# songlab-cal/CherryML

Hardware: AMD Instinct MI355X
Metric: cherry-pairs/sec (whole node) per EM iter (higher is better)
Workload: dtype f64

## Files before the change

### cherryml_amd/csrc/cb_internal.hip.h

```cpp
#pragma once
#include "../../include/cherrybank.h"

#include <hip/hip_runtime.h>

#include <algorithm>
#include <atomic>
#include <chrono>
#include <cmath>
#include <cstdarg>
#include <cstdio>
#include <cstdlib>
#include <cstring>
#include <string>
#include <vector>

int cb_fail(int code, const char *fmt, ...);
#define fail cb_fail

#define HIP_TRY(expr)                                                                   \
  do {                                                                                  \
    hipError_t e_ = (expr);                                                             \
    if (e_ != hipSuccess)                                                               \
      return fail(e_ == hipErrorOutOfMemory ? CB_ENOMEM : CB_EHIP, "%s failed: %s (%s:%d)", \
                  #expr, hipGetErrorString(e_), __FILE__, __LINE__);                    \
  } while (0)

#define CB_REUSE_EIGH 256
int cb_internal_expm_bank(cb_handle h, const double *Q, const double *pi, int flags, double *P);
int cb_internal_set_times(cb_handle h, const double *t_host, int B, const double *t_dev);
struct CbSpectral {
  int S = 0, LD = 0;
  const double *A = nullptr, *U = nullptr, *lam = nullptr, *dsq = nullptr, *sigma = nullptr;
};
int cb_internal_spectral(cb_handle h, CbSpectral *out);

int cb_launch_bank_fused(int variant, int kg, const void *args, int grid, hipStream_t stream, hipEvent_t stop);

#define CB_TB_RS_MAX 24
#define CB_TB_RG_MAX 40
struct CbTimeBasisHost {
  int B = 0, ns = 0, nd = 0, ng = 0;
  double rho_max = 0.0;
  double res_s = 0.0, res_g = 0.0;
  std::vector<int> kind;
  std::vector<int> skel_s, direct, skel_g;
  std::vector<double> tf, tg;
  std::vector<double> Ls, Lg;
};
bool cb_tb_build(int B, const double *t, double rho_max, CbTimeBasisHost &out);
struct CbTbEwArgs {
  int S, LD, B, ns, nd, ng;
  int nsmall;
  const double *Ct;
  const double *Psi;
  const double *A;
  const double *t;
  const double *Ls, *Lg;
  double *Gh;
  float *Gh32;
  double *loss_part;
  double inv_n;
  const unsigned long long *skip;
};
int cb_tb_launch_tables(int LD, int ns, int nd, int ng, const double *tf, const double *tg, const double *lam, double *F, double *E,
                        double *H, const unsigned long long *skip, hipStream_t stream);
#define CB_TB_LDS_MAX (144u << 10)
size_t cb_tb_ew_lds_bytes(int B, int ns, int ng);
bool cb_tb_supported(int B, int LD, int ns, int ng);
int cb_tb_prepare_ew(int B, int ns, int ng, size_t *cache);
int cb_tb_launch_ew(const CbTbEwArgs &a, hipStream_t stream, hipEvent_t stop, int *nparts);

static inline const char *cb_test_hook(const char *name) {
  const char *on = getenv("CB_TEST_HOOKS");
  return (on && on[0] == '1') ? getenv(name) : nullptr;
}
static inline size_t cb_hook_bytes(const char *name, size_t bytes) {
  const char *s = cb_test_hook(name);
  const long long x = s ? atoll(s) : 0;
  return x > 0 ? (size_t)x : bytes;
}

struct CbDevBufs {
  std::vector<void *> ptrs;
  ~CbDevBufs() {
    for (void *p : ptrs)
      if (p) (void)hipFree(p);
  }
  template <typename T>
  T *up(const T *host, size_t count, int &rc) {
    void *q = nullptr;
    if (rc != CB_OK) return nullptr;
    if (hipMalloc(&q, (count ? count : 1) * sizeof(T)) != hipSuccess) {
      rc = fail(CB_ENOMEM, "device allocation failed");
      return nullptr;
    }
    ptrs.push_back(q);
// ... 56 lines not shown
```

### cherryml_amd/csrc/cherrybank.hip

```cpp
#include "cb_internal.hip.h"

#include "common.hip.h"
#include "jacobi_block.hip.h"
#include "jacobi_wave.hip.h"
#include "large_bank.hip.h"
#include "small_bank.hip.h"
#include "train_small.hip.h"
#include "train_large.hip.h"
#include "general_small.hip.h"
#include "general_large.hip.h"
#include "eigh_planned.hip.h"

#define CB_ABI_VERSION 2

static thread_local std::string g_err;

int cb_fail(int code, const char *fmt, ...) {
  char buf[512];
  va_list ap;
  va_start(ap, fmt);
  vsnprintf(buf, sizeof buf, fmt, ap);
  va_end(ap);
  g_err = buf;
  return code;
// ... 204 lines not shown
      return nb;
    });
    h->tb_next_pending = true;
    h->tb_next_epoch = epoch + lead;
  }
  return CB_OK;
}

struct LargeBankForm {
  bool tb = false;
  bool fused = false;
  bool accum = false;
  int kg = 1;
  int n_parts = 1;
  int tiles_k3 = 0;
  int test_no_claim = 0;
  double phi_delta = 0;
};

static LargeBankForm choose_large_form(const cb_bank *h, int B, bool Pd, bool want_grad, bool planned_now) {
  static const int streams = getenv("CB_BANK_STREAMS") ? std::min(4, std::max(1, atoi(getenv("CB_BANK_STREAMS")))) : 1;
  const char *tb_hook = cb_test_hook("CB_BANK_TB"), *fused_hook = cb_test_hook("CB_BANK_FUSED"),
             *unfused_hook = cb_test_hook("CB_BANK_UNFUSED"), *k3_hook = cb_test_hook("CB_BANK_K3"),
             *kg_hook = cb_test_hook("CB_BANK_KG"), *no_claim_hook = cb_test_hook("CB_BANK_TEST_NO_CLAIM"),
             *phi_z_hook = cb_test_hook("CB_PHI_Z");
  const int LD = h->LD, tm = (LD + LG_TM - 1) / LG_TM, tn = (LD + LG_TN - 1) / LG_TN;
  const bool f32 = h->dtype == CB_F32 && !Pd;
  LargeBankForm f;
  const bool form_hooks = fused_hook || unfused_hook || k3_hook || kg_hook || no_claim_hook;
  f.tb = h->sym_counts && !h->per_bucket_products && !h->tb_block && !h->tb_failed && !Pd && want_grad && h->tb_Ls[0] &&
         streams == 1 && (h->dtype == CB_F64 || h->dtype == CB_MIXED) &&
         (tb_hook ? atoi(tb_hook) != 0 : (!form_hooks && B >= CB_TB_MIN_B));
  if (f.tb && planned_now && h->tb.B != B) f.tb = false;
  {
    const size_t nb16 = (size_t)LD / 16, cap = (size_t)B * tm * tn;
    if (nb16 * (nb16 + 1) > cap) f.tb = false;
  }
  f.fused = !Pd && want_grad && !unfused_hook && streams == 1 && h->bank_queue && (fused_hook || B >= CB_BANK_FUSED_MIN_B);
  f.accum = h->sym_counts && !h->per_bucket_products && !Pd && want_grad && h->Yk && streams == 1 && h->dtype == CB_F64 &&
            (k3_hook ? atoi(k3_hook) == 0 : (B >= CB_BANK_SUM_FIRST_MIN_B && h->phi_delta >= 4e-3));
  f.tiles_k3 = f.accum ? 0 : h->sym_counts ? tn * (tn + 1) / 2 : tm * tn;
  f.phi_delta = h->phi_delta;
  if (phi_z_hook) f.phi_delta *= atof(phi_z_hook) / 0.1;
  f.kg = (B < CB_BANK_KG2_MAX_B && !f32) ? 2 : 1;
  if (kg_hook) f.kg = atoi(kg_hook) == 1 ? 1 : 2;
  if (Pd) f.kg = 1;
  if (streams > 1 && h->dtype == CB_F64 && !Pd && want_grad && B >= 4 * streams && !h->comm && !h->profile) f.n_parts = streams;
  f.test_no_claim = no_claim_hook ? 1 : 0;
  return f;
}

struct LargeCall {
  int B;
  const double *t;
  double inv_n;
  double *loss, *dQ, *Pd;
  bool dA_padded, planned_now;
  const unsigned long long *skipw;
  size_t LL;
  int tiles, tiles_k1;
};

template <typename T1, typename TG>
struct BankBufs {
  const T1 *Ut, *A, *F, *Ct;
  TG *Gt, *T;
  const TG *U;
  int variant;
};
template <typename T1, typename TG>
// ... 38 lines not shown
                        hipEvent_t k3_stop) {
  const int LD = h->LD;
  const LossArgs la{h->loss_part, nparts, h->S, h->dsq, h->dirsum, c.inv_n, c.loss, c.skipw};
  const dim3 red_grid((unsigned)((c.LL + 255) / 256) + 1);
  if (f.accum) {
    hipLaunchKernelGGL(ky_reduce_loss<TG>, red_grid, dim3(256), 0, h->stream, src, YArgs{LD, c.B, c.t, h->E, h->Yk}, la);
    K4Args gl{h->S, LD, h->Yk, h->U, h->Lk, nullptr, nullptr, nullptr};
    gl.skip = c.skipw;
    gl.ystride = c.LL;
    launch_sg(h, gl, 0, 0.0, 0.0, nullptr, nullptr, 1 + CB_PHI_TERMS);
    LAUNCH_STOP(k3_stop, kphi_combine<CB_PHI_TERMS>, dim3((unsigned)((c.LL + 255) / 256)), dim3(256), 0, h->stream, LD, h->Lk,
                h->lam, f.phi_delta, h->Mt, c.skipw);
  } else {
    hipLaunchKernelGGL(k3_reduce_loss<TG>, red_grid, dim3(256), 0, h->stream, src, nb, c.LL, h->Mt, sym_ld, la);
  }
  enqueue_k4(h, c, c.skipw, stop_event(h, EV_K4));
  HIP_TRY(hipGetLastError());
  return CB_OK;
}

template <typename TG>
static int enqueue_tb_bank(cb_bank *h, const LargeBankForm &f, const LargeCall &c) {
  constexpr bool mixed = std::is_same_v<TG, float>;
  const CbTimeBasisHost &bas = h->tb;
  const int S = h->S, LD = h->LD, set = h->tb_set, nf = bas.ns + bas.nd, ng = bas.ng;
  const auto bb = bank_bufs<double, TG>(h);
  if (!c.planned_now && cb_tb_launch_tables(LD, bas.ns, bas.nd, ng, h->tb_tf[set], h->tb_tg[set], h->lam, h->F, h->E, h->H,
                                            c.skipw, h->stream) != 0)
    return fail(CB_EHIP, "tb_tables: launch failed");
  double *psi_buf = mixed ? reinterpret_cast<double *>(h->T32) : h->T;
  K1Args<double> k1{S, LD, nf, h->Vc, h->A, h->tb_tf[set], h->F, h->sigma, h->Ct, psi_buf, h->loss_part, c.inv_n, h->dsq, nullptr, c.skipw};
  LAUNCH_STOP(stop_event(h, EV_K1), (k1_pt_loss_gt<double, double, false, 1, true>), dim3(c.tiles_k1 * nf), dim3(LG4_THREADS), 0,
              h->stream, k1);
  const CbTbEwArgs ew{S, LD, c.B, bas.ns, bas.nd, ng, c.B - bas.nd, h->Ct, psi_buf, h->A, c.t, h->tb_Ls[set], h->tb_Lg[set], h->Gt,
                      mixed ? h->Gt32 : nullptr, h->loss_part, c.inv_n, c.skipw};
  int ew_parts = 0;
  if (cb_tb_launch_ew(ew, h->stream, stop_event(h, EV_K2), &ew_parts) != 0) return fail(CB_EHIP, "tb_ew: launch failed");
  if (mixed) launch_cast_f32(h, c, 0);
  const K2Args<TG> k2{LD, bb.Gt, bb.U, bb.T, c.skipw};
  const K3Args<TG> k3{LD, ng, bb.T, bb.U, h->tb_tg[set], h->lam, h->E, h->H, bb.Gt, 1, c.skipw};
  hipLaunchKernelGGL((k2_t_eq_g_u<TG, 1>), dim3(c.tiles * ng), dim3(LG4_THREADS), 0, h->stream, k2);
  LAUNCH_STOP(stop_event(h, EV_K3), (k3_w_phi<TG, 1>), dim3(c.tiles_k1 * ng), dim3(LG4_THREADS), 0, h->stream, k3);
  return enqueue_tail<TG>(h, f, c, bb.Gt, ng, ew_parts, LD, nullptr);
}

template <typename T1, typename TG>
static int enqueue_fused_bank(cb_bank *h, const LargeBankForm &f, const LargeCall &c) {
  const int S = h->S, LD = h->LD, B = c.B;
  const auto bb = bank_bufs<T1, TG>(h);
  const int total = B * (c.tiles_k1 + c.tiles + f.tiles_k3), grid = std::min(h->bank_slots / f.kg, total);
  const int sym = h->sym_counts ? 1 : 0;
  if (h->profile && h->profile_now) h->ev_rec[EV_K1] = h->ev_rec[EV_K2] = false;
  const hipEvent_t bank_stop = stop_event(h, EV_K3);
  static_assert(sizeof(K123Args<float, float>) == sizeof(K123Args<double, double>) &&
                sizeof(K123Args<double, float>) == sizeof(K123Args<double, double>), "one argument block for all");
  const K123Args<T1, TG> a{{S, LD, B, bb.Ut, bb.A, c.t, bb.F, h->sigma, bb.Ct, bb.Gt, h->loss_part, c.inv_n, h->dsq, nullptr, c.skipw},
                           {LD, bb.Gt, bb.U, bb.T, c.skipw},
                           {LD, B, bb.T, bb.U, c.t, h->lam, h->E, h->H, bb.Gt, sym, c.skipw},
                           {h->bank_queue, B, c.tiles_k1, c.tiles, f.tiles_k3, h->bank_claims, f.test_no_claim}};
  auto *dst = reinterpret_cast<K123Args<T1, TG> *>(h->bank_args);
  hipLaunchKernelGGL((lg_tables<K123Args<T1, TG>>), dim3((unsigned)(((size_t)B * LD + 255) / 256)), dim3(256), 0, h->stream, LD, B,
                     c.t, h->lam, h->sigma, h->F, h->E, h->H, a, dst, grid);
  if (std::is_same_v<TG, float>) launch_cast_f32(h, c, (size_t)B * LD);
  if (cb_launch_bank_fused(bb.variant, f.kg, dst, grid, h->stream, bank_stop) != 0) return fail(CB_EHIP, "k123_bank: launch failed");
  return enqueue_tail<TG>(h, f, c, f.accum ? bb.T : bb.Gt, B, B * c.tiles_k1, h->sym_counts ? LD : 0, nullptr);
}

// ... 447 lines not shown
```

### cherryml_amd/csrc/create_host.hip.h

```cpp
#pragma once
__global__ void prep_counts(int S, int B, const double *C, double *n, double *inv_n, double *ones,
                            double *dirsum) {
  extern __shared__ double sm[];
  const int l = blockIdx.x;
  const double *Cl = C + (size_t)l * B * S * S;
  for (int e = threadIdx.x; e < S * S; e += blockDim.x) {
    double acc = 0.0;
    for (int b = 0; b < B; ++b) acc += Cl[(size_t)b * S * S + e];
    sm[e] = acc;
  }
  __syncthreads();
  for (int k = threadIdx.x; k < S; k += blockDim.x) {
    double cs = 0.0, rs = 0.0;
    for (int i = 0; i < S; ++i) {
      cs += sm[i * S + k];
      rs += sm[k * S + i];
    }
    dirsum[(size_t)l * S + k] = cs - rs;
  }
  if (threadIdx.x == 0) {
    double tot = 0.0;
    for (int e = 0; e < S * S; ++e) tot += sm[e];
    n[l] = tot;
    inv_n[l] = 1.0 / tot;
// ... 253 lines not shown
      (void)hipMemsetAsync(flag, 0, sizeof(int), h->stream);
      hipLaunchKernelGGL(small_sym_check, dim3((unsigned)nmat), dim3(256), 0, h->stream, S, Cdev, flag);
      int hf = 1;
      if (hipMemcpyAsync(&hf, flag, sizeof hf, hipMemcpyDeviceToHost, h->stream) == hipSuccess &&
          hipStreamSynchronize(h->stream) == hipSuccess)
        h->sym_counts = hf == 0 && !cb_test_hook("CB_NO_SYM");
      (void)hipMemsetAsync(flag, 0, sizeof(int), h->stream);
    }
  } else {
    const size_t LL = (size_t)h->LD * h->LD;
    const int tiles = ((h->LD + LG_TM - 1) / LG_TM) * ((h->LD + LG_TN - 1) / LG_TN);
    h->k3_chunk = 4;
    h->k3_nchunks = (B + h->k3_chunk - 1) / h->k3_chunk;
    double *tot = nullptr;
    const bool f32 = h->dtype == CB_F32, mixed = h->dtype == CB_MIXED, narrow = f32 || mixed;
    const size_t per_bucket = (expm_only || narrow) ? 0 : (size_t)Bl * LL;
    const size_t per_bucket32 = narrow ? (size_t)Bl * LL : 0;
    bool ok = dev_alloc(h, &h->Ct, mixed ? (size_t)Bl * LL : per_bucket) == CB_OK && dev_alloc(h, &tot, SS) == CB_OK &&
              dev_alloc(h, &h->Ct32, f32 ? per_bucket32 : 0) == CB_OK && dev_alloc(h, &h->Gt32, per_bucket32) == CB_OK &&
              dev_alloc(h, &h->T32, per_bucket32) == CB_OK && dev_alloc(h, &h->Uf, narrow ? LL : 0) == CB_OK &&
              dev_alloc(h, &h->Utf, narrow ? LL : 0) == CB_OK && dev_alloc(h, &h->Af, narrow ? LL : 0) == CB_OK &&
              dev_alloc(h, &h->Ff, narrow ? (size_t)B * h->LD : 0) == CB_OK &&
              dev_alloc(h, &h->A, LL) == CB_OK && dev_alloc(h, &h->dsq, h->LD) == CB_OK &&
              dev_alloc(h, &h->Gc, LL) == CB_OK && dev_alloc(h, &h->Vc, LL) == CB_OK &&
              dev_alloc(h, &h->Gc2, LL) == CB_OK && dev_alloc(h, &h->gx, 12 * LL + (size_t)h->LD + 16 + 3 * 256 + 8) == CB_OK &&
              dev_alloc(h, &h->U, LL) == CB_OK && dev_alloc(h, &h->lam, h->LD) == CB_OK &&
              dev_alloc(h, &h->sigma, 8) == CB_OK && dev_alloc(h, &h->off_bits, 64) == CB_OK &&
              dev_alloc(h, &h->F, (size_t)B * h->LD) == CB_OK &&
              dev_alloc(h, &h->E, (size_t)B * h->LD) == CB_OK &&
              dev_alloc(h, &h->H, (size_t)B * h->LD) == CB_OK &&
              dev_alloc(h, &h->Gt, per_bucket) == CB_OK &&
              dev_alloc(h, &h->T, per_bucket) == CB_OK &&
              dev_alloc(h, &h->Mt, LL) == CB_OK && dev_alloc(h, &h->X, LL) == CB_OK &&
              dev_alloc(h, &h->loss_part, (size_t)B * tiles) == CB_OK &&
              dev_alloc(h, &h->Yk, expm_only ? 0 : (1 + CB_PHI_TERMS) * LL) == CB_OK &&
              dev_alloc(h, &h->Lk, expm_only ? 0 : (1 + CB_PHI_TERMS) * LL) == CB_OK;
    if (ok && !expm_only && !f32)
      for (int k = 0; k < 2 && ok; ++k)
        ok = dev_alloc(h, &h->tb_Ls[k], (size_t)Bl * CB_TB_RS_MAX) == CB_OK && dev_alloc(h, &h->tb_Lg[k], (size_t)Bl * CB_TB_RG_MAX) == CB_OK &&
             dev_alloc(h, &h->tb_tf[k], Bl) == CB_OK && dev_alloc(h, &h->tb_tg[k], Bl) == CB_OK;
    if (!ok) {
      free_tmp();
      return cleanup(CB_ENOMEM);
    }
    {
      void *q = nullptr;
      if (hipHostMalloc(&q, 8 * sizeof(unsigned long long), hipHostMallocCoherent | hipHostMallocMapped) == hipSuccess) {
        h->poll = (unsigned long long *)q;
        memset(q, 0, 8 * sizeof(unsigned long long));
      } else {
        (void)hipGetLastError();
      }
    }
    if (!expm_only) {
      int dev = 0, cus = 0;
      if (hipGetDevice(&dev) != hipSuccess || hipDeviceGetAttribute(&cus, hipDeviceAttributeMultiprocessorCount, dev) != hipSuccess)
        cus = 256;
      h->bank_slots = 4 * std::max(cus, 1);
      h->bank_claims = (h->bank_slots + LG_NQ - 1) / LG_NQ;
      if (dev_alloc(h, &h->bank_queue, (size_t)LG_NQ + 2 * (size_t)B + (size_t)LG_NQ * h->bank_claims) != CB_OK ||
          dev_alloc(h, &h->bank_args, sizeof(K123Args<double, double>)) != CB_OK) {
        free_tmp();
        return cleanup(CB_ENOMEM);
      }
    }
    if (!expm_only) {
    hipLaunchKernelGGL(prep_counts_large_tot, dim3((unsigned)((SS + 255) / 256)), dim3(256), 0,
                       h->stream, S, B, Cdev, tot);
    hipLaunchKernelGGL(prep_counts_large_fin, dim3(1), dim3(256), 0, h->stream, S, tot, h->n_dev,
                       h->inv_n, h->ones, h->dirsum);
    const int nt32 = (h->LD + 31) / 32;
    if (f32) hipLaunchKernelGGL(lg_transpose_pad<float>, dim3(nt32, nt32, Bl), dim3(32, 8), 0, h->stream, S, h->LD,
                                Cdev, h->Ct32, src_idx);
    else hipLaunchKernelGGL(lg_transpose_pad<double>, dim3(nt32, nt32, Bl), dim3(32, 8), 0, h->stream, S, h->LD,
                            Cdev, h->Ct, src_idx);
    {
      int *flag = reinterpret_cast<int *>(h->status);
      (void)hipMemsetAsync(flag, 0, sizeof(int), h->stream);
      if (f32) hipLaunchKernelGGL(lg_sym_check<float>, dim3(nt32, nt32, Bl), dim3(32, 32), 0, h->stream, h->LD, h->Ct32, flag);
      else hipLaunchKernelGGL(lg_sym_check<double>, dim3(nt32, nt32, Bl), dim3(32, 32), 0, h->stream, h->LD, h->Ct, flag);
      int hf = 1;
      if (hipMemcpyAsync(&hf, flag, sizeof hf, hipMemcpyDeviceToHost, h->stream) == hipSuccess &&
          hipStreamSynchronize(h->stream) == hipSuccess)
        h->sym_counts = hf == 0 && !cb_test_hook("CB_NO_SYM");
    }
    }
  }
  h->n_host.resize(L);
  hipError_t e = hipMemcpyAsync(h->n_host.data(), h->n_dev, L * sizeof(double), hipMemcpyDeviceToHost,
                                h->stream);
  if (e == hipSuccess) e = hipStreamSynchronize(h->stream);
  if (Ctmp) (void)hipFree(Ctmp);
  if (e != hipSuccess) return cleanup(fail(CB_EHIP, "cb_create: upload failed: %s", hipGetErrorString(e)));
  e = hipGetLastError();
  if (e != hipSuccess) return cleanup(fail(CB_EHIP, "cb_create: kernel failed: %s", hipGetErrorString(e)));
  for (int l = 0; l < L; ++l)
    if (!(h->n_host[l] > 0.0) || !std::isfinite(h->n_host[l]))
      return cleanup(fail(CB_ENUMERIC, "cb_create: site %d has total count %g", l, h->n_host[l]));
  *out = h;
  return CB_OK;
#undef TRY_ALLOC
#undef TRY_HIP
}

extern "C" void cb_destroy(cb_handle h) {
  if (!h) return;
  if (h->tb_next_pending) (void)h->tb_next.get();
  (void)hipSetDevice(h->dev);
  if (h->own_stream) (void)hipStreamSynchronize(h->own_stream);
  for (hipEvent_t e : h->ev)
    if (e) (void)hipEventDestroy(e);
  for (hipEvent_t e : h->ev2)
    if (e) (void)hipEventDestroy(e);
  for (void *p : h->allocs) (void)hipFree(p);
  for (double *p : h->ws_ptr)
    if (p) (void)hipFree(p);
  if (h->pin) (void)hipHostFree(h->pin);
  if (h->poll) (void)hipHostFree(h->poll);
// ... 13 lines not shown
```

### cherryml_amd/csrc/handle_host.hip.h

```cpp
#pragma once
#include <hip/hip_ext.h>
#include <future>
struct EighSlot {
  int cap = 12;
  int nsq = 0;
  int band_after = 0;
  int so = 0;
  int expect_run = 1, expect_order = 12, expect_sq = 2;
};
struct EighPlan {
  int lead_band = 1;
  int nslots = 0;
  EighSlot slot[EC_MAXREC];
};
struct cb_bank {
  int dev = 0, S = 0, L = 0, B = 0;
  int B_cap = 0;
  hipStream_t xstream[3] = {};
  hipEvent_t ev_fork = nullptr, ev_join[3] = {};
  int tr_epochs = 0;
  uint64_t tr_sig = 0;
  int last_form = 0;
  double tr_pow_b1 = 1.0, tr_pow_b2 = 1.0;
  int dtype = CB_F64;
// ... 31 lines not shown
         *sigma = nullptr, *F = nullptr, *E = nullptr, *H = nullptr, *Gt = nullptr, *T = nullptr,
         *Mt_part = nullptr, *Mt = nullptr, *X = nullptr, *loss_part = nullptr;
  float *Ct32 = nullptr, *Gt32 = nullptr, *T32 = nullptr, *Uf = nullptr, *Utf = nullptr, *Af = nullptr, *Ff = nullptr;
  unsigned long long *off_bits = nullptr;
  unsigned long long *poll = nullptr;
  unsigned long long poll_seq = 0;
  unsigned long long *ectl = nullptr, *epin = nullptr;
  double *epart = nullptr;
  bool begin_folded = false;
  double *sigma_home = nullptr;
  double *sigma2 = nullptr;
  unsigned long long eseq = 0;
  bool planned_unavailable = false;
  int planned_solves = 0, planned_stalls = 0;
  long long record_spins = 0;
  std::vector<double> epoch_seconds;
  EighPlan eplan;
  int k3_chunk = 0, k3_nchunks = 0;
  double *Yk = nullptr, *Lk = nullptr;
  double phi_delta = 0.0;
  unsigned int *bank_queue = nullptr;
  unsigned char *bank_args = nullptr;
  int bank_slots = 0;
  int bank_claims = 0;
  bool bank_fused = false;
  int bank_kg = 1;
  bool bank_accum = false;
  CbTimeBasisHost tb;
  int tb_set = 0;
  double *tb_Ls[2] = {}, *tb_Lg[2] = {}, *tb_tf[2] = {}, *tb_tg[2] = {};
  std::future<CbTimeBasisHost> tb_next;
  bool tb_next_pending = false;
  int tb_next_epoch = 0;
  size_t tb_ew_lds[4] = {0, 0, 0, 0};
  int tb_builds = 0, tb_stale_epochs = 0;
  bool tb_failed = false;
  bool tb_block = false;
  bool bank_tb = false;
  int last_sweeps = 0;
  double *gn_scratch = nullptr, *gn_partial = nullptr;
  int gn_nw = 0;
  struct {
    double *Qn = nullptr, *QT = nullptr, *colsum = nullptr, *alpha = nullptr, *R = nullptr, *RT = nullptr, *E = nullptr,
           *ET = nullptr, *G = nullptr, *GT = nullptr, *Xbar = nullptr, *lpart = nullptr;
    int *nsq = nullptr;
    int cap_slots = 0;
  } gl;
  std::vector<double> t_host, t_live_host;
  bool have_prev = false;
  double *ws_ptr[16] = {};
  size_t ws_cap[16] = {};
  char *pin = nullptr;
  size_t pin_cap = 0, pin_off = 0;
  bool profile = false;
  int profile_every = 1;
  bool profile_now = false;
  hipEvent_t ev[CB_T_COUNT + 1] = {};
  bool ev_rec[CB_T_COUNT + 1] = {};
  double t_sum[CB_T_COUNT] = {};
  int t_calls = 0;
  bool t_pending = false;
  hipEvent_t ev2[CB_T_COUNT + 1] = {};
  bool ev_rec2[CB_T_COUNT + 1] = {};
  bool t_pending2 = false;
};

// ... 102 lines not shown
```

### cherryml_amd/csrc/tbasis.hip.h

```cpp
#pragma once
#include "cb_internal.hip.h"
#include "common.hip.h"
#include <hip/hip_ext.h>

namespace tbasis {

typedef long double ld;

static inline ld g_phi2(ld x) {
  if (fabsl(x) < 0.5L) {
    ld p = 1.0L;
    for (int k = 24; k >= 3; --k) p = 1.0L + p * x / (ld)k;
    return 0.5L * p;
  }
  return (expm1l(x) - x) / (x * x);
}

static inline ld dot4(const ld *a, const ld *b, int n) {
  ld s0 = 0.0L, s1 = 0.0L, s2 = 0.0L, s3 = 0.0L;
  int i = 0;
  for (; i + 3 < n; i += 4) {
    s0 += a[i] * b[i];
    s1 += a[i + 1] * b[i + 1];
    s2 += a[i + 2] * b[i + 2];
    s3 += a[i + 3] * b[i + 3];
  }
  for (; i < n; ++i) s0 += a[i] * b[i];
  return (s0 + s1) + (s2 + s3);
}

static int id_rows(int B, int N, const std::vector<ld> &F, int Rmax, ld tol, std::vector<int> &skel, std::vector<ld> &L, ld &resid) {
  std::vector<ld> W(F), Q((size_t)Rmax * N, 0.0L), Cq((size_t)B * Rmax, 0.0L), q(N);
  skel.clear();
  ld scale = 0.0L;
  int R = 0;
// ... 123 lines not shown
    out.res_g = (double)res;
    out.skel_g = sk;
    for (int b = 0; b < B; ++b)
      for (int r = 0; r < R; ++r)
        out.Lg[(size_t)b * CB_TB_RG_MAX + r] = (double)(L[(size_t)b * R + r] * (ld)t[b] / (ld)t[sk[r]]);
  }
  for (int r = 0; r < out.ns; ++r) out.tf.push_back(t[out.skel_s[r]]);
  for (int r = 0; r < out.nd; ++r) out.tf.push_back(t[out.direct[r]]);
  for (int r = 0; r < out.ng; ++r) out.tg.push_back(t[out.skel_g[r]]);
  return true;
}

__global__ void tb_tables(int LD, int ns, int nd, int ng, const double *__restrict__ tf, const double *__restrict__ tg,
                          const double *__restrict__ lam, double *__restrict__ F, double *__restrict__ E, double *__restrict__ H,
                          const unsigned long long *skip) {
  if (skip && *skip != 0ull) return;
  const int idx = blockIdx.x * blockDim.x + threadIdx.x;
  const int nf = ns + nd;
  if (idx >= (nf + ng) * LD) return;
  const int r = idx / LD, k = idx - r * LD;
  if (r < nf) {
    const double t = tf[r], x = t * lam[k];
    F[idx] = r < ns ? phi2(x) / (t * t) : exp(x);
  } else {
    const double x = tg[r - nf] * lam[k];
    E[idx - nf * LD] = exp(x);
    H[idx - nf * LD] = exp(0.5 * x);
  }
}

template <int RS, int RG>
struct TbEwLds {
  static constexpr int SS = RS + 1, SG = RG + 2;
  int BP, LS, LG, TT, LT, RED, TOTAL;
  __host__ __device__ explicit TbEwLds(int B) {
    BP = (B + 15) & ~15;
    LS = 0;
    LG = LS + BP * SS;
    TT = LG + BP * SG;
    LT = TT + BP;
    RED = LT + 256;
    TOTAL = RED + 16;
  }
};

template <int RS, int RG>
__device__ __forceinline__ void tb_ew_step(int b0, int j, int k, int nsm, const double *sLs, const double *sLg, const double *sT,
                                           const double *ltab, const double (&psi)[RS / 4], double a_e, double dl, double inv_n,
                                           const double (&c)[4], const double (&pd)[4], d4 (&D)[RG / 16], double &loss, int &bad) {
  typedef TbEwLds<RS, RG> Lds;
  const bool any_small = b0 < nsm, any_direct = b0 + 16 > nsm;
  double P[4];
  if (any_small) {
    d4 acc = {0.0, 0.0, 0.0, 0.0};
#ifndef TB_NO_FWD
#pragma unroll
    for (int q = 0; q < RS / 4; ++q) acc = mfma_f64(sLs[(b0 + j) * Lds::SS + 4 * q + k], psi[q], acc);
#endif
#pragma unroll
    for (int m = 0; m < 4; ++m) {
      const double t = sT[b0 + k + 4 * m];
      P[m] = fma(t, fma(t, acc[m], a_e), dl);
    }
    if (any_direct) {
#pragma unroll
      for (int m = 0; m < 4; ++m) P[m] = (b0 + k + 4 * m < nsm) ? P[m] : pd[m];
    }
  } else {
#pragma unroll
    for (int m = 0; m < 4; ++m) P[m] = pd[m];
  }
  double g[4];
#pragma unroll
  for (int m = 0; m < 4; ++m) {
    const double cv = c[m];
    bad |= (!(P[m] >= 1e-300) && cv != 0.0) ? 1 : 0;
    const double Pu = fmax(P[m], 1e-300);
#ifdef TB_NO_LOG
    loss = fma(-cv, Pu, loss);
    g[m] = (-cv * inv_n) * Pu;
#else
    loss = fma(-cv, fast_log_table_unchecked(Pu, ltab), loss);
    g[m] = (-cv * inv_n) * fast_rcp(Pu);
#endif
  }
#ifdef TB_NO_BWD
#pragma unroll
  for (int m = 0; m < 4; ++m) D[0][m] += g[m];
#else
#pragma unroll
  for (int m = 0; m < 4; ++m) {
    const double *w = sLg + (b0 + 4 * m + k) * Lds::SG + j;
#pragma unroll
    for (int q = 0; q < RG / 16; ++q) D[q] = mfma_f64(w[16 * q], g[m], D[q]);
  }
#endif
}

template <int RS, int RG, int NWAVE, bool SYM>
__global__ __launch_bounds__(NWAVE * 64, 4) void tb_ew(CbTbEwArgs a) {
  constexpr int NT = NWAVE * 64;
  typedef TbEwLds<RS, RG> Lds;
  extern __shared__ double smem[];
  if (a.skip && *a.skip != 0ull) return;
  const Lds o(a.B);
  double *sLs = smem + o.LS, *sLg = smem + o.LG, *sT = smem + o.TT, *ltab = smem + o.LT, *sred = smem + o.RED;
  const int tid = threadIdx.x;
  for (int i = tid; i < o.BP * RS; i += NT) {
    const int b = i / RS, r = i - b * RS;
    sLs[b * Lds::SS + r] = b < a.B ? a.Ls[(size_t)b * CB_TB_RS_MAX + r] : 0.0;
  }
  for (int i = tid; i < o.BP * RG; i += NT) {
    const int b = i / RG, r = i - b * RG;
    sLg[b * Lds::SG + r] = (b < a.B && r < CB_TB_RG_MAX) ? a.Lg[(size_t)b * CB_TB_RG_MAX + r] : 0.0;
  }
  for (int i = tid; i < o.BP; i += NT) sT[i] = i < a.B ? a.t[i] : 0.0;
  fast_log_table_fill(ltab, tid, NT);
  __syncthreads();
  const size_t LL = (size_t)a.LD * a.LD;
  const int wave = tid >> 6, lane = tid & 63, j = lane & 15, k = lane >> 4;
  size_t e;
  bool live;
  double lossw = 1.0;
  if (SYM) {
    const int nb = a.LD / 16, item = (int)blockIdx.x * NWAVE + wave, blk = item >> 4, rr = item & 15;
    int I = 0, rest = blk;
    while (I < nb && rest >= nb - I) {
      rest -= nb - I;
      ++I;
    }
    live = I < nb;
    const int J = I + rest;
    e = live ? ((size_t)(16 * I + rr) * a.LD + 16 * J + j) : 0;
    lossw = J > I ? 2.0 : 1.0;
  } else {
    e = ((size_t)blockIdx.x * NWAVE + wave) * 16 + j;
    live = e < LL;
  }
  const size_t ec = live ? e : 0;
  const int row = (int)(ec / a.LD), col = (int)(ec - (size_t)row * a.LD);
  const double *__restrict__ Psi = a.Psi + ec;
  double psi[RS / 4];
#pragma unroll
  for (int q = 0; q < RS / 4; ++q) psi[q] = (4 * q + k < a.ns) ? Psi[(size_t)(4 * q + k) * LL] : 0.0;
  const double a_e = a.A[ec], dl = row == col ? 1.0 : 0.0;
  d4 D[RG / 16];
#pragma unroll
  for (int q = 0; q < RG / 16; ++q) D[q] = d4{0.0, 0.0, 0.0, 0.0};
  double loss = 0.0;
  int bad = 0;
  const int nsm = a.nsmall, B = a.B;
  const unsigned plane = (unsigned)(LL * sizeof(double));
  const __amdgpu_buffer_rsrc_t rc = __builtin_amdgcn_make_buffer_rsrc(const_cast<double *>(a.Ct), 0, 0x7fffffff, 0x00027000);
  const __amdgpu_buffer_rsrc_t rp = __builtin_amdgcn_make_buffer_rsrc(const_cast<double *>(a.Psi + (size_t)a.ns * LL), 0, 0x7fffffff, 0x00027000);
  const int eoff = (int)(ec * sizeof(double));
  int voff[4];
#pragma unroll
  for (int m = 0; m < 4; ++m) voff[m] = (int)((unsigned)(k + 4 * m) * plane) + eoff;
  auto load = [&](int b0, double (&cc)[4], double (&pp)[4]) {
    if (b0 >= B) return;
#ifdef TB_NO_LOAD
    for (int m = 0; m < 4; ++m) cc[m] = 1.0 + b0 + m, pp[m] = 0.5;
    return;
#endif
    if (b0 + 16 <= B) {
#pragma unroll
      for (int m = 0; m < 4; ++m)
        cc[m] = __builtin_bit_cast(double, __builtin_amdgcn_raw_buffer_load_b64(rc, voff[m], (int)((unsigned)b0 * plane), 0));
      if (b0 >= nsm) {
#pragma unroll
        for (int m = 0; m < 4; ++m)
          pp[m] = __builtin_bit_cast(double, __builtin_amdgcn_raw_buffer_load_b64(rp, voff[m], (int)((unsigned)(b0 - nsm) * plane), 0));
        return;
      }
      if (b0 + 16 <= nsm) return;
    } else {
#pragma unroll
      for (int m = 0; m < 4; ++m) {
        const bool in = b0 + k + 4 * m < B;
        const double v = __builtin_bit_cast(double, __builtin_amdgcn_raw_buffer_load_b64(rc, in ? voff[m] + (int)((unsigned)b0 * plane) : eoff, 0, 0));
        cc[m] = in ? v : 0.0;
      }
    }
#pragma unroll
    for (int m = 0; m < 4; ++m) {
      const int b = b0 + k + 4 * m;
      const bool in = b >= nsm && b < B;
      const double v = __builtin_bit_cast(double, __builtin_amdgcn_raw_buffer_load_b64(rp, (int)((unsigned)(in ? b - nsm : 0) * plane) + eoff, 0, 0));
      pp[m] = in ? v : 1.0;
    }
  };
  double c0[4] = {0.0, 0.0, 0.0, 0.0}, c1[4] = {0.0, 0.0, 0.0, 0.0}, p0[4] = {1.0, 1.0, 1.0, 1.0}, p1[4] = {1.0, 1.0, 1.0, 1.0};
  load(0, c0, p0);
  for (int b0 = 0; b0 < B; b0 += 32) {
    load(b0 + 16, c1, p1);
    tb_ew_step<RS, RG>(b0, j, k, nsm, sLs, sLg, sT, ltab, psi, a_e, dl, a.inv_n, c0, p0, D, loss, bad);
    if (b0 + 16 >= B) break;
    load(b0 + 32, c0, p0);
    tb_ew_step<RS, RG>(b0 + 16, j, k, nsm, sLs, sLg, sT, ltab, psi, a_e, dl, a.inv_n, c1, p1, D, loss, bad);
  }
  if (live) {
    if (a.Gh32) {
      float *__restrict__ Gh = a.Gh32 + e;
#pragma unroll
      for (int q = 0; q < RG / 16; ++q)
#pragma unroll
        for (int r = 0; r < 4; ++r) {
          const int rr = 16 * q + k + 4 * r;
          if (rr < a.ng) Gh[(size_t)rr * LL] = (float)D[q][r];
        }
    } else {
      double *__restrict__ Gh = a.Gh + e;
#pragma unroll
      for (int q = 0; q < RG / 16; ++q)
#pragma unroll
        for (int r = 0; r < 4; ++r) {
          const int rr = 16 * q + k + 4 * r;
          if (rr < a.ng) Gh[(size_t)rr * LL] = D[q][r];
        }
    }
  } else {
    loss = 0.0;
    bad = 0;
  }
  if (bad) loss = NAN;
  loss = wave_sum(loss) * lossw;
  if (lane == 0) sred[wave] = loss;
  __syncthreads();
  if (tid == 0) {
    double s = 0.0;
    for (int w = 0; w < NWAVE; ++w) s += sred[w];
    a.loss_part[blockIdx.x] = s;
  }
}

template <typename T>
__global__ __launch_bounds__(256) void tb_mirror(int LD, T *__restrict__ Gh, const unsigned long long *skip) {
  __shared__ T tile[16][17];
  if (skip && *skip != 0ull) return;
  const int nb = LD / 16;
  int I = 0, rest = (int)blockIdx.x;
  while (rest >= nb - 1 - I) {
    rest -= nb - 1 - I;
    ++I;
  }
  const int J = I + 1 + rest, r = threadIdx.x >> 4, c = threadIdx.x & 15;
  T *G = Gh + (size_t)blockIdx.y * LD * LD;
  tile[r][c] = G[(size_t)(16 * I + r) * LD + 16 * J + c];
  __syncthreads();
  G[(size_t)(16 * J + r) * LD + 16 * I + c] = tile[c][r];
}

int cb_tb_launch_tables(int LD, int ns, int nd, int ng, const double *tf, const double *tg, const double *lam, double *F, double *E,
                        double *H, const unsigned long long *skip, hipStream_t stream) {
  const int n = (ns + nd + ng) * LD;
  hipLaunchKernelGGL(tb_tables, dim3((unsigned)((n + 255) / 256)), dim3(256), 0, stream, LD, ns, nd, ng, tf, tg, lam, F, E, H, skip);
  return hipGetLastError() == hipSuccess ? 0 : -1;
}

bool cb_tb_supported(int B, int LD, int ns, int ng) {
  return ns <= CB_TB_RS_MAX && ng <= CB_TB_RG_MAX && LD % 16 == 0 && cb_tb_ew_lds_bytes(B, ns, ng) <= CB_TB_LDS_MAX &&
         (double)(B + 32) * (double)LD * (double)LD * 8.0 < 2147483648.0;
}

size_t cb_tb_ew_lds_bytes(int B, int ns, int ng) {
  const int RS = ns <= 16 ? 16 : 24, RG = ng <= 32 ? 32 : 48;
  const int BP = (B + 15) & ~15;
  return ((size_t)BP * (RS + 1 + RG + 2 + 1) + 256 + 16) * sizeof(double);
}

int cb_tb_prepare_ew(int B, int ns, int ng, size_t *cache) {
#define TB_PREP(RS_, RG_, slot_)                                                                                         \
  do {                                                                                                                   \
    const size_t lds = (size_t)TbEwLds<RS_, RG_>(B).TOTAL * sizeof(double);                                              \
    if (lds > cache[slot_]) {                                                                                            \
      if (hipFuncSetAttribute(reinterpret_cast<const void *>(tb_ew<RS_, RG_, 8, true>), hipFuncAttributeMaxDynamicSharedMemorySize, (int)lds) != hipSuccess) { \
        (void)hipGetLastError();                                                                                         \
        return -1;                                                                                                       \
      }                                                                                                                  \
      cache[slot_] = lds;                                                                                                \
    }                                                                                                                    \
  } while (0)
  if (ns <= 16 && ng <= 32) TB_PREP(16, 32, 0);
  else if (ns <= 16) TB_PREP(16, 48, 1);
  else if (ng <= 32) TB_PREP(24, 32, 2);
  else TB_PREP(24, 48, 3);
#undef TB_PREP
  return 0;
}

int cb_tb_launch_ew(const CbTbEwArgs &a, hipStream_t stream, hipEvent_t stop, int *nparts) {
  if (!cb_tb_supported(a.B, a.LD, a.ns, a.ng)) return -1;
  const int nb = a.LD / 16, nblk = nb * (nb + 1) / 2;
  const unsigned grid = (unsigned)(nblk * 2);
  if (nparts) *nparts = (int)grid;
#define TB_GO(RS_, RG_)                                                                                                  \
  do {                                                                                                                   \
    const size_t lds = (size_t)TbEwLds<RS_, RG_>(a.B).TOTAL * sizeof(double);                                            \
    hipLaunchKernelGGL((tb_ew<RS_, RG_, 8, true>), dim3(grid), dim3(512), lds, stream, a);                               \
  } while (0)
  if (a.ns <= 16 && a.ng <= 32) TB_GO(16, 32);
  else if (a.ns <= 16) TB_GO(16, 48);
  else if (a.ng <= 32) TB_GO(24, 32);
  else TB_GO(24, 48);
#undef TB_GO
  if (nb > 1) {
    const dim3 mg((unsigned)(nb * (nb - 1) / 2), (unsigned)a.ng);
    if (a.Gh32) {
      if (stop) hipExtLaunchKernelGGL(tb_mirror<float>, mg, dim3(256), 0, stream, nullptr, stop, 0, a.LD, a.Gh32, a.skip);
      else hipLaunchKernelGGL(tb_mirror<float>, mg, dim3(256), 0, stream, a.LD, a.Gh32, a.skip);
    } else {
      if (stop) hipExtLaunchKernelGGL(tb_mirror<double>, mg, dim3(256), 0, stream, nullptr, stop, 0, a.LD, a.Gh, a.skip);
      else hipLaunchKernelGGL(tb_mirror<double>, mg, dim3(256), 0, stream, a.LD, a.Gh, a.skip);
    }
  } else if (stop) {
    (void)hipEventRecord(stop, stream);
  }
  return hipGetLastError() == hipSuccess ? 0 : -1;
}
```

Before: 1.535 billion.

## Pack symmetric count blocks contiguously and fuse mirror write into tb_ew

Adds a one-time packing kernel that reorders the per-bucket count tensor into contiguous runs per upper-triangular 16x16 block, so the time-basis elementwise kernel reads counts with short strides instead of plane-strided loads. The separate tb_mirror kernel is removed; each workgroup now transposes its off-diagonal gradient tile through LDS and writes the mirrored block directly, saving a launch and a global read-back. It also drops a gate that disabled the time-basis path for small tile counts, and enlarges loss_part to fit. The cost is extra device memory for the packed copy, a larger LDS footprint, and extra barriers in the kernel epilogue.

```diff
diff --git a/cherryml_amd/csrc/cb_internal.hip.h b/cherryml_amd/csrc/cb_internal.hip.h
--- a/cherryml_amd/csrc/cb_internal.hip.h
+++ b/cherryml_amd/csrc/cb_internal.hip.h
@@ -52,6 +52,7 @@
   int S, LD, B, ns, nd, ng;
   int nsmall;
   const double *Ct;
+  const double *Cpk;
   const double *Psi;
   const double *A;
   const double *t;
@@ -62,6 +63,8 @@
   double inv_n;
   const unsigned long long *skip;
 };
+size_t cb_tb_packed_doubles(int B, int LD);
+int cb_tb_pack_counts(int B, int LD, const double *Ct, double *Cpk, hipStream_t stream);
 int cb_tb_launch_tables(int LD, int ns, int nd, int ng, const double *tf, const double *tg, const double *lam, double *F, double *E,
                         double *H, const unsigned long long *skip, hipStream_t stream);
 #define CB_TB_LDS_MAX (144u << 10)
diff --git a/cherryml_amd/csrc/cherrybank.hip b/cherryml_amd/csrc/cherrybank.hip
--- a/cherryml_amd/csrc/cherrybank.hip
+++ b/cherryml_amd/csrc/cherrybank.hip
@@ -260,10 +260,6 @@
          streams == 1 && (h->dtype == CB_F64 || h->dtype == CB_MIXED) &&
          (tb_hook ? atoi(tb_hook) != 0 : (!form_hooks && B >= CB_TB_MIN_B));
   if (f.tb && planned_now && h->tb.B != B) f.tb = false;
-  {
-    const size_t nb16 = (size_t)LD / 16, cap = (size_t)B * tm * tn;
-    if (nb16 * (nb16 + 1) > cap) f.tb = false;
-  }
   f.fused = !Pd && want_grad && !unfused_hook && streams == 1 && h->bank_queue && (fused_hook || B >= CB_BANK_FUSED_MIN_B);
   f.accum = h->sym_counts && !h->per_bucket_products && !Pd && want_grad && h->Yk && streams == 1 && h->dtype == CB_F64 &&
             (k3_hook ? atoi(k3_hook) == 0 : (B >= CB_BANK_SUM_FIRST_MIN_B && h->phi_delta >= 4e-3));
@@ -368,7 +364,8 @@
   K1Args<double> k1{S, LD, nf, h->Vc, h->A, h->tb_tf[set], h->F, h->sigma, h->Ct, psi_buf, h->loss_part, c.inv_n, h->dsq, nullptr, c.skipw};
   LAUNCH_STOP(stop_event(h, EV_K1), (k1_pt_loss_gt<double, double, false, 1, true>), dim3(c.tiles_k1 * nf), dim3(LG4_THREADS), 0,
               h->stream, k1);
-  const CbTbEwArgs ew{S, LD, c.B, bas.ns, bas.nd, ng, c.B - bas.nd, h->Ct, psi_buf, h->A, c.t, h->tb_Ls[set], h->tb_Lg[set], h->Gt,
+  const double *Cpk = (c.B == h->Bl && !cb_test_hook("CB_TB_PLANE_MAJOR")) ? h->Cpk : nullptr;
+  const CbTbEwArgs ew{S, LD, c.B, bas.ns, bas.nd, ng, c.B - bas.nd, h->Ct, Cpk, psi_buf, h->A, c.t, h->tb_Ls[set], h->tb_Lg[set], h->Gt,
                       mixed ? h->Gt32 : nullptr, h->loss_part, c.inv_n, c.skipw};
   int ew_parts = 0;
   if (cb_tb_launch_ew(ew, h->stream, stop_event(h, EV_K2), &ew_parts) != 0) return fail(CB_EHIP, "tb_ew: launch failed");
diff --git a/cherryml_amd/csrc/create_host.hip.h b/cherryml_amd/csrc/create_host.hip.h
--- a/cherryml_amd/csrc/create_host.hip.h
+++ b/cherryml_amd/csrc/create_host.hip.h
@@ -309,7 +309,7 @@
               dev_alloc(h, &h->Gt, per_bucket) == CB_OK &&
               dev_alloc(h, &h->T, per_bucket) == CB_OK &&
               dev_alloc(h, &h->Mt, LL) == CB_OK && dev_alloc(h, &h->X, LL) == CB_OK &&
-              dev_alloc(h, &h->loss_part, (size_t)B * tiles) == CB_OK &&
+              dev_alloc(h, &h->loss_part, std::max((size_t)B * tiles, ((size_t)h->LD / 16) * ((size_t)h->LD / 16 + 1))) == CB_OK &&
               dev_alloc(h, &h->Yk, expm_only ? 0 : (1 + CB_PHI_TERMS) * LL) == CB_OK &&
               dev_alloc(h, &h->Lk, expm_only ? 0 : (1 + CB_PHI_TERMS) * LL) == CB_OK;
     if (ok && !expm_only && !f32)
@@ -361,6 +361,16 @@
           hipStreamSynchronize(h->stream) == hipSuccess)
         h->sym_counts = hf == 0 && !cb_test_hook("CB_NO_SYM");
     }
+    const size_t npk = cb_tb_packed_doubles(Bl, h->LD);
+    if (h->sym_counts && !f32 && !h->per_bucket_products && h->tb_Ls[0] && npk && (double)npk * 8.0 < 2147483648.0) {
+      void *q = nullptr;
+      if (hipMalloc(&q, npk * sizeof(double) + 64) == hipSuccess) {
+        h->allocs.push_back(q);
+        if (cb_tb_pack_counts(Bl, h->LD, h->Ct, static_cast<double *>(q), h->stream) == 0) h->Cpk = static_cast<double *>(q);
+      } else {
+        (void)hipGetLastError();
+      }
+    }
     }
   }
   h->n_host.resize(L);
diff --git a/cherryml_amd/csrc/handle_host.hip.h b/cherryml_amd/csrc/handle_host.hip.h
--- a/cherryml_amd/csrc/handle_host.hip.h
+++ b/cherryml_amd/csrc/handle_host.hip.h
@@ -87,6 +87,7 @@
   std::future<CbTimeBasisHost> tb_next;
   bool tb_next_pending = false;
   int tb_next_epoch = 0;
+  double *Cpk = nullptr;
   size_t tb_ew_lds[4] = {0, 0, 0, 0};
   int tb_builds = 0, tb_stale_epochs = 0;
   bool tb_failed = false;
diff --git a/cherryml_amd/csrc/tb_pack_layout.h b/cherryml_amd/csrc/tb_pack_layout.h
--- /dev/null
+++ b/cherryml_amd/csrc/tb_pack_layout.h
@@ -0,0 +1,26 @@
+#pragma once
+#include <stddef.h>
+
+#if defined(__HIPCC__)
+#define TB_PK_HD __host__ __device__
+#else
+#define TB_PK_HD
+#endif
+
+TB_PK_HD inline int tb_pack_blocks(int nb) { return nb * (nb + 1) / 2; }
+TB_PK_HD inline size_t tb_pack_doubles(int B, int LD) { return (size_t)tb_pack_blocks(LD / 16) * 256 * (size_t)B; }
+TB_PK_HD inline bool tb_pack_block(int nb, int blk, int *I, int *J) {
+  int i = 0, rest = blk;
+  while (i < nb && rest >= nb - i) {
+    rest -= nb - i;
+    ++i;
+  }
+  *I = i;
+  *J = i + rest;
+  return i < nb;
+}
+TB_PK_HD inline size_t tb_pack_run(int item, int B) { return (size_t)item * 16 * (size_t)B; }
+TB_PK_HD inline size_t tb_pack_index(int item, int B, int b, int c) { return tb_pack_run(item, B) + (size_t)b * 16 + c; }
+TB_PK_HD inline size_t tb_pack_source(int LD, int I, int J, int r, int b, int c) {
+  return ((size_t)b * LD + 16 * I + r) * LD + 16 * J + c;
+}
diff --git a/cherryml_amd/csrc/tbasis.hip.h b/cherryml_amd/csrc/tbasis.hip.h
--- a/cherryml_amd/csrc/tbasis.hip.h
+++ b/cherryml_amd/csrc/tbasis.hip.h
@@ -1,6 +1,7 @@
 #pragma once
 #include "cb_internal.hip.h"
 #include "common.hip.h"
+#include "tb_pack_layout.h"
 #include <hip/hip_ext.h>
 
 namespace tbasis {
@@ -190,6 +191,7 @@
 template <int RS, int RG>
 struct TbEwLds {
   static constexpr int SS = RS + 1, SG = RG + 2;
+  static constexpr int MIR_ROW = 24, MIR_PLANE = 8 * MIR_ROW + 16, MIR = 16 * MIR_PLANE;
   int BP, LS, LG, TT, LT, RED, TOTAL;
   __host__ __device__ explicit TbEwLds(int B) {
     BP = (B + 15) & ~15;
@@ -198,7 +200,7 @@
     TT = LG + BP * SG;
     LT = TT + BP;
     RED = LT + 256;
-    TOTAL = RED + 16;
+    TOTAL = RED + 16 > MIR ? RED + 16 : MIR;
   }
 };
 
@@ -255,9 +257,11 @@
 #endif
 }
 
-template <int RS, int RG, int NWAVE, bool SYM>
-__global__ __launch_bounds__(NWAVE * 64, 4) void tb_ew(CbTbEwArgs a) {
+template <int RS, int RG, int NWAVE, bool SYM, bool PK>
+__device__ __forceinline__ void tb_ew_body(const CbTbEwArgs &a) {
   constexpr int NT = NWAVE * 64;
+  static_assert(SYM || !PK, "the packed counts belong to the symmetric form");
+  static_assert(!SYM || NWAVE == 8, "the mirror's thread map: eight rows of a block per workgroup");
   typedef TbEwLds<RS, RG> Lds;
   extern __shared__ double smem[];
   if (a.skip && *a.skip != 0ull) return;
@@ -280,15 +284,11 @@
   size_t e;
   bool live;
   double lossw = 1.0;
+  int item = 0, I = 0, J = 0;
   if (SYM) {
-    const int nb = a.LD / 16, item = (int)blockIdx.x * NWAVE + wave, blk = item >> 4, rr = item & 15;
-    int I = 0, rest = blk;
-    while (I < nb && rest >= nb - I) {
-      rest -= nb - I;
-      ++I;
-    }
-    live = I < nb;
-    const int J = I + rest;
+    item = (int)blockIdx.x * NWAVE + wave;
+    const int rr = item & 15;
+    live = tb_pack_block(a.LD / 16, item >> 4, &I, &J);
     e = live ? ((size_t)(16 * I + rr) * a.LD + 16 * J + j) : 0;
     lossw = J > I ? 2.0 : 1.0;
   } else {
@@ -309,12 +309,21 @@
   int bad = 0;
   const int nsm = a.nsmall, B = a.B;
   const unsigned plane = (unsigned)(LL * sizeof(double));
-  const __amdgpu_buffer_rsrc_t rc = __builtin_amdgcn_make_buffer_rsrc(const_cast<double *>(a.Ct), 0, 0x7fffffff, 0x00027000);
   const __amdgpu_buffer_rsrc_t rp = __builtin_amdgcn_make_buffer_rsrc(const_cast<double *>(a.Psi + (size_t)a.ns * LL), 0, 0x7fffffff, 0x00027000);
   const int eoff = (int)(ec * sizeof(double));
   int voff[4];
 #pragma unroll
   for (int m = 0; m < 4; ++m) voff[m] = (int)((unsigned)(k + 4 * m) * plane) + eoff;
+  const __amdgpu_buffer_rsrc_t rc = __builtin_amdgcn_make_buffer_rsrc(const_cast<double *>(PK ? a.Cpk : a.Ct), 0, 0x7fffffff, 0x00027000);
+  const int crun = PK ? (int)(tb_pack_index(live ? item : 0, B, 0, j) * sizeof(double)) : eoff, cvo = crun + k * 128;
+  auto load_c = [&](int m, int b0) {
+    if constexpr (PK) return __builtin_bit_cast(double, __builtin_amdgcn_raw_buffer_load_b64(rc, cvo + 512 * m, b0 * 128, 0));
+    else return __builtin_bit_cast(double, __builtin_amdgcn_raw_buffer_load_b64(rc, voff[m], (int)((unsigned)b0 * plane), 0));
+  };
+  auto load_c_checked = [&](int m, int b0, bool in) {
+    if constexpr (PK) return __builtin_bit_cast(double, __builtin_amdgcn_raw_buffer_load_b64(rc, in ? cvo + 512 * m + b0 * 128 : crun, 0, 0));
+    else return __builtin_bit_cast(double, __builtin_amdgcn_raw_buffer_load_b64(rc, in ? voff[m] + (int)((unsigned)b0 * plane) : eoff, 0, 0));
+  };
   auto load = [&](int b0, double (&cc)[4], double (&pp)[4]) {
     if (b0 >= B) return;
 #ifdef TB_NO_LOAD
@@ -324,7 +333,7 @@
     if (b0 + 16 <= B) {
 #pragma unroll
       for (int m = 0; m < 4; ++m)
-        cc[m] = __builtin_bit_cast(double, __builtin_amdgcn_raw_buffer_load_b64(rc, voff[m], (int)((unsigned)b0 * plane), 0));
+        cc[m] = load_c(m, b0);
       if (b0 >= nsm) {
 #pragma unroll
         for (int m = 0; m < 4; ++m)
@@ -336,7 +345,7 @@
 #pragma unroll
       for (int m = 0; m < 4; ++m) {
         const bool in = b0 + k + 4 * m < B;
-        const double v = __builtin_bit_cast(double, __builtin_amdgcn_raw_buffer_load_b64(rc, in ? voff[m] + (int)((unsigned)b0 * plane) : eoff, 0, 0));
+        const double v = load_c_checked(m, b0, in);
         cc[m] = in ? v : 0.0;
       }
     }
@@ -381,6 +390,28 @@
     loss = 0.0;
     bad = 0;
   }
+  if (SYM && live && J > I) {
+    __syncthreads();
+    const int r0 = ((int)blockIdx.x * NWAVE) & 15, c8 = tid & 7, jr = (tid >> 3) & 15, ps = tid >> 7;
+    const size_t dst = (size_t)(16 * J + jr) * a.LD + 16 * I + r0 + c8;
+#pragma unroll
+    for (int q = 0; q < RG / 16; ++q) {
+      if (16 * q >= a.ng) break;
+#pragma unroll
+      for (int r = 0; r < 4; ++r) smem[(k + 4 * r) * Lds::MIR_PLANE + wave * Lds::MIR_ROW + j] = D[q][r];
+      __syncthreads();
+#pragma unroll
+      for (int i = 0; i < 4; ++i) {
+        const int p = ps + 4 * i, rr = 16 * q + p;
+        const double v = smem[p * Lds::MIR_PLANE + c8 * Lds::MIR_ROW + jr];
+        if (rr < a.ng) {
+          if (a.Gh32) a.Gh32[(size_t)rr * LL + dst] = (float)v;
+          else a.Gh[(size_t)rr * LL + dst] = v;
+        }
+      }
+      __syncthreads();
+    }
+  }
   if (bad) loss = NAN;
   loss = wave_sum(loss) * lossw;
   if (lane == 0) sred[wave] = loss;
@@ -392,21 +423,13 @@
   }
 }
 
-template <typename T>
-__global__ __launch_bounds__(256) void tb_mirror(int LD, T *__restrict__ Gh, const unsigned long long *skip) {
-  __shared__ T tile[16][17];
-  if (skip && *skip != 0ull) return;
-  const int nb = LD / 16;
-  int I = 0, rest = (int)blockIdx.x;
-  while (rest >= nb - 1 - I) {
-    rest -= nb - 1 - I;
-    ++I;
-  }
-  const int J = I + 1 + rest, r = threadIdx.x >> 4, c = threadIdx.x & 15;
-  T *G = Gh + (size_t)blockIdx.y * LD * LD;
-  tile[r][c] = G[(size_t)(16 * I + r) * LD + 16 * J + c];
-  __syncthreads();
-  G[(size_t)(16 * J + r) * LD + 16 * I + c] = tile[c][r];
+template <int RS, int RG, int NWAVE, bool SYM>
+__global__ __launch_bounds__(NWAVE * 64, 4) void tb_ew(CbTbEwArgs a) {
+  tb_ew_body<RS, RG, NWAVE, SYM, true>(a);
+}
+template <int RS, int RG, int NWAVE, bool SYM>
+__global__ __launch_bounds__(NWAVE * 64, 4) void tb_ew_planes(CbTbEwArgs a) {
+  tb_ew_body<RS, RG, NWAVE, SYM, false>(a);
 }
 
 int cb_tb_launch_tables(int LD, int ns, int nd, int ng, const double *tf, const double *tg, const double *lam, double *F, double *E,
@@ -416,34 +439,52 @@
   return hipGetLastError() == hipSuccess ? 0 : -1;
 }
 
+__global__ __launch_bounds__(256) void tb_pack_counts(int LD, int B, const double *__restrict__ Ct, double *__restrict__ Cpk) {
+  int I, J;
+  if (!tb_pack_block(LD / 16, (int)blockIdx.x, &I, &J)) return;
+  const int b = (int)blockIdx.y, r = threadIdx.x >> 4, c = threadIdx.x & 15;
+  Cpk[tb_pack_index(16 * (int)blockIdx.x + r, B, b, c)] = Ct[tb_pack_source(LD, I, J, r, b, c)];
+}
+
+size_t cb_tb_packed_doubles(int B, int LD) { return (LD > 0 && LD % 16 == 0 && B > 0) ? tb_pack_doubles(B, LD) : 0; }
+
+int cb_tb_pack_counts(int B, int LD, const double *Ct, double *Cpk, hipStream_t stream) {
+  if (cb_tb_packed_doubles(B, LD) == 0 || B > 65535) return -1;
+  hipLaunchKernelGGL(tb_pack_counts, dim3((unsigned)tb_pack_blocks(LD / 16), (unsigned)B), dim3(256), 0, stream, LD, B, Ct, Cpk);
+  return hipGetLastError() == hipSuccess ? 0 : -1;
+}
+
 bool cb_tb_supported(int B, int LD, int ns, int ng) {
   return ns <= CB_TB_RS_MAX && ng <= CB_TB_RG_MAX && LD % 16 == 0 && cb_tb_ew_lds_bytes(B, ns, ng) <= CB_TB_LDS_MAX &&
-         (double)(B + 32) * (double)LD * (double)LD * 8.0 < 2147483648.0;
+         (double)(B + 32) * (double)LD * (double)LD * 8.0 < 2147483648.0 && (double)tb_pack_doubles(B, LD) * 8.0 < 2147483648.0;
 }
 
 size_t cb_tb_ew_lds_bytes(int B, int ns, int ng) {
-  const int RS = ns <= 16 ? 16 : 24, RG = ng <= 32 ? 32 : 48;
-  const int BP = (B + 15) & ~15;
-  return ((size_t)BP * (RS + 1 + RG + 2 + 1) + 256 + 16) * sizeof(double);
+  return (ns <= 16 ? (ng <= 32 ? TbEwLds<16, 32>(B).TOTAL : TbEwLds<16, 48>(B).TOTAL)
+                   : (ng <= 32 ? TbEwLds<24, 32>(B).TOTAL : TbEwLds<24, 48>(B).TOTAL)) * sizeof(double);
+}
+
+typedef void (*TbEwKernel)(CbTbEwArgs);
+static TbEwKernel tb_ew_kernel(int ns, int ng, bool packed, int *slot) {
+  *slot = (ns <= 16 ? 0 : 2) + (ng <= 32 ? 0 : 1);
+  if (ns <= 16 && ng <= 32) return packed ? tb_ew<16, 32, 8, true> : tb_ew_planes<16, 32, 8, true>;
+  if (ns <= 16) return packed ? tb_ew<16, 48, 8, true> : tb_ew_planes<16, 48, 8, true>;
+  if (ng <= 32) return packed ? tb_ew<24, 32, 8, true> : tb_ew_planes<24, 32, 8, true>;
+  return packed ? tb_ew<24, 48, 8, true> : tb_ew_planes<24, 48, 8, true>;
 }
 
 int cb_tb_prepare_ew(int B, int ns, int ng, size_t *cache) {
-#define TB_PREP(RS_, RG_, slot_)                                                                                         \
-  do {                                                                                                                   \
-    const size_t lds = (size_t)TbEwLds<RS_, RG_>(B).TOTAL * sizeof(double);                                              \
-    if (lds > cache[slot_]) {                                                                                            \
-      if (hipFuncSetAttribute(reinterpret_cast<const void *>(tb_ew<RS_, RG_, 8, true>), hipFuncAttributeMaxDynamicSharedMemorySize, (int)lds) != hipSuccess) { \
-        (void)hipGetLastError();                                                                                         \
-        return -1;                                                                                                       \
-      }                                                                                                                  \
-      cache[slot_] = lds;                                                                                                \
-    }                                                                                                                    \
-  } while (0)
-  if (ns <= 16 && ng <= 32) TB_PREP(16, 32, 0);
-  else if (ns <= 16) TB_PREP(16, 48, 1);
-  else if (ng <= 32) TB_PREP(24, 32, 2);
-  else TB_PREP(24, 48, 3);
-#undef TB_PREP
+  int slot = 0;
+  (void)tb_ew_kernel(ns, ng, false, &slot);
+  const size_t lds = cb_tb_ew_lds_bytes(B, ns, ng);
+  if (lds <= cache[slot]) return 0;
+  for (const bool packed : {false, true})
+    if (hipFuncSetAttribute(reinterpret_cast<const void *>(tb_ew_kernel(ns, ng, packed, &slot)),
+                            hipFuncAttributeMaxDynamicSharedMemorySize, (int)lds) != hipSuccess) {
+      (void)hipGetLastError();
+      return -1;
+    }
+  cache[slot] = lds;
   return 0;
 }
 
@@ -452,27 +493,10 @@
   const int nb = a.LD / 16, nblk = nb * (nb + 1) / 2;
   const unsigned grid = (unsigned)(nblk * 2);
   if (nparts) *nparts = (int)grid;
-#define TB_GO(RS_, RG_)                                                                                                  \
-  do {                                                                                                                   \
-    const size_t lds = (size_t)TbEwLds<RS_, RG_>(a.B).TOTAL * sizeof(double);                                            \
-    hipLaunchKernelGGL((tb_ew<RS_, RG_, 8, true>), dim3(grid), dim3(512), lds, stream, a);                               \
-  } while (0)
-  if (a.ns <= 16 && a.ng <= 32) TB_GO(16, 32);
-  else if (a.ns <= 16) TB_GO(16, 48);
-  else if (a.ng <= 32) TB_GO(24, 32);
-  else TB_GO(24, 48);
-#undef TB_GO
-  if (nb > 1) {
-    const dim3 mg((unsigned)(nb * (nb - 1) / 2), (unsigned)a.ng);
-    if (a.Gh32) {
-      if (stop) hipExtLaunchKernelGGL(tb_mirror<float>, mg, dim3(256), 0, stream, nullptr, stop, 0, a.LD, a.Gh32, a.skip);
-      else hipLaunchKernelGGL(tb_mirror<float>, mg, dim3(256), 0, stream, a.LD, a.Gh32, a.skip);
-    } else {
-      if (stop) hipExtLaunchKernelGGL(tb_mirror<double>, mg, dim3(256), 0, stream, nullptr, stop, 0, a.LD, a.Gh, a.skip);
-      else hipLaunchKernelGGL(tb_mirror<double>, mg, dim3(256), 0, stream, a.LD, a.Gh, a.skip);
-    }
-  } else if (stop) {
-    (void)hipEventRecord(stop, stream);
-  }
+  int slot = 0;
+  const TbEwKernel kern = tb_ew_kernel(a.ns, a.ng, a.Cpk != nullptr, &slot);
+  const size_t lds = cb_tb_ew_lds_bytes(a.B, a.ns, a.ng);
+  if (stop) hipExtLaunchKernelGGL(kern, dim3(grid), dim3(512), lds, stream, nullptr, stop, 0, a);
+  else hipLaunchKernelGGL(kern, dim3(grid), dim3(512), lds, stream, a);
   return hipGetLastError() == hipSuccess ? 0 : -1;
 }
```

After: 1.557 billion, median of 6. Within noise of the previous version (+1.4%).
